# Mamo1031/Multimodal-MTRSSM

Hardware: AMD Instinct MI355X
Metric: seq-steps/s (BxT) MoPoE-MRSSM train step (higher is better)
Workload: dtype bf16x2-split, fp32 accumulate; 1 GPU; BASELINE configs[1]: MoPoE-MRSSM train step, B=64/GPU T=50 deter=200 stoch=30, vision 1x64x64 + audio 1x128x32 + action 4; global_batch=64, seq_len=50, parallelism=dp1, hidden=200, embed=256, categoricals_x_classes=6x5, residual_blocks=3, activation=ELU, optimizer=AdamW lr 1e-3 + clip 10 (fused HIP), params=4151600, streams=1, launch=eager (host enqueues every launch), backend=none, rccl_ranks=0, collective_ranks=0, noise=uniforms keyed by global batch row (parallel.GlobalRowNoise)

## Files before the change

include/mtrssm.h:

```cpp
#ifndef MTRSSM_H
#define MTRSSM_H

#include <stddef.h>
#include <stdint.h>

#ifdef __cplusplus
extern "C" {
#endif

#define MTRSSM_VERSION 100

#define MTRSSM_OK 0
#define MTRSSM_EINVAL (-1)
#define MTRSSM_ELAUNCH (-2)
#define MTRSSM_ELDS (-3)

#define MTRSSM_ACT_IDENTITY 0
#define MTRSSM_ACT_RELU 1
#define MTRSSM_ACT_ELU 2
#define MTRSSM_ACT_TANH 3

int mtrssm_version(void);
const char* mtrssm_last_error(void);
const char* mtrssm_last_kernel(void);
// ... 388 lines not shown
                                 int64_t workspace_a_bytes, const MtrssmConvGeom* gb, const float* ab, const float* srcb, float* dwpb,
                                 float* dbiasb, void* workspace_b, int64_t workspace_b_bytes, int32_t defer, void* stream);
int mtrssm_conv_weight_grad_src_bias(const MtrssmConvGeom* g, const float* a, const float* src, int32_t pre_act_a, float* dwp,
                                     float* dsrc_bias, void* workspace, int64_t workspace_bytes, int32_t defer, void* stream);
int64_t mtrssm_conv_weight_grad_workspace_bytes(const MtrssmConvGeom* g, int32_t pre_act_a);
int mtrssm_unpack_conv_grads(const int64_t* table, int32_t count, int32_t blocks_per_entry, void* stream);
int mtrssm_convt_quad_supported(const MtrssmConvGeom* g4);
int mtrssm_convt_quad(const MtrssmConvGeom* ga4, const float* srca, const uint16_t* const* wqa4, const float* biasa, const float* actgrada,
                      float* outa, const MtrssmConvGeom* gb4, const float* srcb, const uint16_t* const* wqb4, const float* biasb,
                      const float* actgradb, float* outb, void* stream);
int mtrssm_convt_k4s2_thin(int32_t N, int32_t C, int32_t Hs, int32_t Ws, int32_t Cout, const float* src, const float* w,
                           const float* bias, int32_t pre_act, int32_t act, float* out, void* stream);
int mtrssm_convt_k4s2_band_supported(int32_t N, int32_t C, int32_t Hs, int32_t Ws, int32_t Cout);
int mtrssm_convt_k4s2_band(int32_t N, int32_t C, int32_t Hs, int32_t Ws, int32_t Cout, const float* src, const float* w,
                           const float* bias, int32_t pre_act, int32_t act, float* out, void* stream);
int mtrssm_conv_tgather_thin(int32_t N, int32_t O, int32_t Hs, int32_t Ws, int32_t Cout, int32_t KH, int32_t KW, int32_t stride, int32_t pad,
                             int32_t Ho, int32_t Wo, const float* y, const float* w, const float* bias, int32_t pre_act, int32_t act,
                             const float* actgrad_in, const float* add_in, float* out, void* stream);
int mtrssm_channel_sum(const float* x, int32_t N, int32_t C, int32_t HW, float* out, void* stream);

int mtrssm_episode_gather(const float* store, const int64_t* idx, const float* noise, int64_t n_episodes, int64_t B, int64_t T,
                          int64_t Tfull, int64_t E, float std_, float* input, float* target, void* stream);
int mtrssm_episode_gather_window(const float* store, const int64_t* idx, const int32_t* start, const float* noise, int64_t n_episodes,
                                 int64_t B, int64_t T, int64_t Tfull, int64_t E, float std_, float* input, float* target, void* stream);
int mtrssm_episode_gather_ragged(const float* store, const int64_t* idx, const int32_t* start, const int32_t* lengths, const float* noise,
                                 int64_t n_episodes, int64_t B, int64_t T, int64_t Tfull, int64_t E, float std_, float* input, float* target,
                                 int32_t* valid_out, void* stream);
int mtrssm_episode_gather_seeded(const float* store, const int64_t* idx, const int32_t* start, const int32_t* lengths, int32_t* valid_out,
                                 uint32_t key0, uint32_t key1, uint32_t epoch, int64_t n_episodes, int64_t B, int64_t T, int64_t Tfull,
                                 int64_t E, float std_, float* input, float* target, void* stream);
// ... 184 lines not shown
```

multimodal_mtrssm_amd/_lib.py:

```python

from __future__ import annotations

import ctypes as C
import os
from pathlib import Path

import torch
from torch import Tensor

_HERE = Path(__file__).resolve().parent
LIB_PATH = _HERE / "libmtrssm_hip.so"

ACT_IDS = {"Identity": 0, "ReLU": 1, "ELU": 2, "Tanh": 3}

_f = C.c_float
_i = C.c_int32
_p = C.c_void_p


def _struct(name: str, fields: list[tuple[str, type]]) -> type:
    return type(name, (C.Structure,), {"_fields_": fields})


def _ptrs(*names: str) -> list[tuple[str, type]]:
# ... 44 lines not shown
    "sv_l1", "sv_h1", "sv_la", "sv_lv", "expert_logw", "modality"))
MmtrssmBwdWeights = _struct("MtrssmMmtrssmBwdWeights", _ptrs(
    "wxl_s_t", "wdl", "wxh_t", "wdh", "wl1", "wh1", "wlp2", "wa2", "wv2", "whp2", "whq2"))
MmtrssmBwdIO = _struct("MtrssmMmtrssmBwdIO", _ptrs(
    "deter_l0", "deter_h0", "deter_l", "deter_h", "prior_logits_l", "prior_logits_h", "post_logits_l", "post_logits_h",
    "sv_l1", "sv_h1", "sv_la", "sv_lv",
    "g_deter_l", "g_deter_h", "g_hidden_l", "g_hidden_h", "g_post_stoch_l", "g_post_stoch_h", "g_prior_stoch_l",
    "g_prior_stoch_h", "g_post_logits_l", "g_post_logits_h", "g_prior_logits_l", "g_prior_logits_h", "g_kl_l", "g_kl_h",
    "g_deter_l0", "g_deter_h0", "g_hidden_l0", "g_hidden_h0", "g_stoch_l0", "g_stoch_h0",
    "d_ul", "d_uh", "d_zl1", "d_zh1", "d_lpl", "d_la", "d_lv", "d_lph", "d_lqh", "expert_logw", "g_expert_logw", "modality"))

ConvGeom = _struct("MtrssmConvGeom", [(n, _i) for n in (
    "N", "C", "Hs", "Ws", "C2", "Cpad", "KH", "KW", "SS", "TS", "OFFY", "OFFX", "Hq", "Wq", "OS", "QY", "QX", "Ho", "Wo",
    "Cout", "CoutPad", "pre_act", "act", "mfma_split")])

Gemm = _struct("MtrssmGemm", _ptrs("A", "B", "C", "bias", "zgrad", "colsum") + [(n, _i) for n in (
    "M", "N", "R", "lda", "ldb", "ldc", "ldz", "a_rmajor", "b_rmajor", "act_a", "act_b", "act_out", "act_z", "accumulate", "split_r")]
    + [("tickets", _p), ("n_tickets", _i), ("mfma_split", _i)])

ElboSchedule = _struct("MtrssmElboSchedule", [(n, _f) for n in ("c0", "c1", "free0", "free1", "w_a", "w_v", "beta_start", "warmup")])

STATE_MAX = 6
StateTable = _struct("MtrssmStateTable", [
    ("count", _i), ("width", _i * STATE_MAX), ("src_stride", C.c_int64 * STATE_MAX), ("src", _p * STATE_MAX), ("alt", _p * STATE_MAX),
    ("dst", _p * STATE_MAX)])

PANEL_COLUMNS = {"prior": 0, "observation": 1, "posterior": 2, "error": 3}
PanelGeom = _struct("MtrssmPanelGeom", [(n, _i) for n in ("N", "T", "Ca", "Ha", "Wa", "Cv", "Hv", "Wv", "scale", "gap", "bar", "label", "frame0")]
                    + [("columns", _i * 4), ("n_columns", _i), ("blank_unseen", _i)])

SYMBOLS: dict[str, tuple[type | None, list[type]]] = {
# ... 39 lines not shown
    "mtrssm_residual_bwd1x1": (C.c_int, [C.POINTER(ConvGeom), _p, _p, _p, _p, _p, _p, _p, C.c_int64, _i, _p]),
    "mtrssm_conv_weight_grad_src_bias_supported": (C.c_int, [C.POINTER(ConvGeom), _i]),
    "mtrssm_conv_weight_grad_src_bias": (C.c_int, [C.POINTER(ConvGeom), _p, _p, _i, _p, _p, _p, C.c_int64, _i, _p]),
    "mtrssm_conv_weight_grad_reduce": (C.c_int, [_p]),
    "mtrssm_conv_weight_grad_workspace_bytes": (C.c_int64, [C.POINTER(ConvGeom), _i]),
    "mtrssm_residual_bwd1x1_pair_supported": (C.c_int, [C.POINTER(ConvGeom), C.POINTER(ConvGeom)]),
    "mtrssm_residual_bwd1x1_pair": (C.c_int, [C.POINTER(ConvGeom), _p, _p, _p, _p, _p, _p, _p, C.c_int64,
                                              C.POINTER(ConvGeom), _p, _p, _p, _p, _p, _p, _p, C.c_int64, _i, _p]),
    "mtrssm_conv_weight_grad_pair_supported": (C.c_int, [C.POINTER(ConvGeom), C.POINTER(ConvGeom)]),
    "mtrssm_conv_weight_grad_pair": (C.c_int, [C.POINTER(ConvGeom), _p, _p, _p, _p, _p, C.c_int64,
                                               C.POINTER(ConvGeom), _p, _p, _p, _p, _p, C.c_int64, _i, _p]),
    "mtrssm_channel_sum": (C.c_int, [_p, _i, _i, _i, _p, _p]),
    "mtrssm_convt_k4s2_thin": (C.c_int, [_i, _i, _i, _i, _i, _p, _p, _p, _i, _i, _p, _p]),
    "mtrssm_convt_k4s2_band_supported": (C.c_int, [_i, _i, _i, _i, _i]),
    "mtrssm_convt_k4s2_band": (C.c_int, [_i, _i, _i, _i, _i, _p, _p, _p, _i, _i, _p, _p]),
    "mtrssm_convt_quad_supported": (C.c_int, [C.POINTER(ConvGeom)]),
    "mtrssm_convt_quad": (C.c_int, [C.POINTER(ConvGeom), _p, C.POINTER(C.c_void_p), _p, _p, _p, C.POINTER(ConvGeom), _p, C.POINTER(C.c_void_p),
                                    _p, _p, _p, _p]),
    "mtrssm_conv_tgather_thin": (C.c_int, [_i] * 11 + [_p, _p, _p, _i, _i, _p, _p, _p, _p]),
    "mtrssm_episode_gather": (C.c_int, [_p, _p, _p, C.c_int64, C.c_int64, C.c_int64, C.c_int64, C.c_int64, _f, _p, _p, _p]),
    "mtrssm_episode_gather_window": (C.c_int, [_p, _p, _p, _p, C.c_int64, C.c_int64, C.c_int64, C.c_int64, C.c_int64, _f, _p, _p, _p]),
    "mtrssm_state_select": (C.c_int, [C.POINTER(StateTable), _p, C.c_int64, _p]),
    "mtrssm_state_save": (C.c_int, [C.POINTER(StateTable), C.c_int64, C.c_int64, _p]),
    "mtrssm_state_save_at": (C.c_int, [C.POINTER(StateTable), _p, C.c_int64, C.c_int64, _p]),
    "mtrssm_episode_gather_ragged": (C.c_int, [_p, _p, _p, _p, _p, C.c_int64, C.c_int64, C.c_int64, C.c_int64, C.c_int64, _f, _p, _p, _p, _p]),
    "mtrssm_episode_gather_seeded": (C.c_int, [_p, _p, _p, _p, _p, C.c_uint32, C.c_uint32, C.c_uint32, C.c_int64, C.c_int64, C.c_int64, C.c_int64,
                                               C.c_int64, _f, _p, _p, _p]),
    "mtrssm_step_mask_ragged": (C.c_int, [_p, _p, C.c_int64, C.c_int64, C.c_int64, _f, _f, C.c_int64, C.c_int64, _p, _p, _p, _p, _p, _p, _p, _p]),
    "mtrssm_step_mask_forecast": (C.c_int, [_p, _p, _p, C.c_int64, C.c_int64, C.c_int64, _f, _f, C.c_int64, C.c_int64, C.c_int64, C.c_int64, _p, _p, _p,
                                            _p, _p, _p, _p, _p, _p]),
# ... 174 lines not shown
```

multimodal_mtrssm_amd/cnn.py:

```python

from __future__ import annotations

from typing import Any

import torch
from torch import Tensor, nn

from multimodal_mtrssm_amd import _lib
from multimodal_mtrssm_amd.linear import SPLIT_MIN_FLOPS, linear, linear_group
from multimodal_mtrssm_amd.conv import (
    gemm_pieces,
    conv2d,
    conv2d_pair,
    conv_transpose2d,
    conv_transpose2d_pair,
    residual_block,
    residual_block_pair,
)


def _act(name: str) -> nn.Module:
    return getattr(nn, name)()


def _cfg(config: Any) -> dict[str, Any]:
    return dict(config) if isinstance(config, dict) else dict(vars(config))


def _conv(x: Tensor, m: nn.Conv2d, *, pre_act: bool, act: int, coords: Tensor | None = None) -> Tensor:
    return conv2d(x, m.weight, m.bias, stride=m.stride[0], padding=m.padding[0], pre_act=pre_act, act=act, coords=coords)
# ... 39 lines not shown


def _conv_pair(xa: Tensor, ma: nn.Conv2d, ca: Tensor | None, xb: Tensor, mb: nn.Conv2d, cb: Tensor | None, *, pre_act: bool,
               act_a: int, act_b: int) -> tuple[Tensor, Tensor]:
    if _same_layer(ma, mb) and act_a == act_b:
        return conv2d_pair((xa, ma.weight, ma.bias, ma.stride[0], ma.padding[0], pre_act, act_a, ca),
                           (xb, mb.weight, mb.bias, mb.stride[0], mb.padding[0], pre_act, act_b, cb))
    return _conv(xa, ma, pre_act=pre_act, act=act_a, coords=ca), _conv(xb, mb, pre_act=pre_act, act=act_b, coords=cb)


def encode_pair(enc_a: "Encoder", enc_b: "Encoder", xa: Tensor, xb: Tensor) -> tuple[Tensor, Tensor]:
    lead_a, lead_b = xa.shape[:-3], xb.shape[:-3]
    xa, ca = enc_a.prepare(xa)
    xb, cb = enc_b.prepare(xb)
    if len(enc_a.convs) == len(enc_b.convs) and (enc_a.res_in is None) == (enc_b.res_in is None):
        for i, (ma, mb) in enumerate(zip(enc_a.convs, enc_b.convs, strict=True)):
            xa, xb = _conv_pair(xa, ma, ca if i == 0 else None, xb, mb, cb if i == 0 else None, pre_act=i > 0, act_a=enc_a.act_id,
                                act_b=enc_b.act_id)
        if enc_a.res_in is not None:
            xa, xb = _conv_pair(xa, enc_a.res_in, None, xb, enc_b.res_in, None, pre_act=True, act_a=enc_a.act_id, act_b=enc_b.act_id)
    else:
        xa, xb = enc_a.stem_convs(xa, ca), enc_b.stem_convs(xb, cb)
    xa, xb = _res_pair(enc_a.res, enc_b.res, xa, xb)
    return enc_a.head(xa, lead_a), enc_b.head(xb, lead_b)


def decode_pair(dec_a: "Decoder", dec_b: "Decoder", fa: Tensor, fb: Tensor, *, raw: bool = False) -> tuple[Tensor, Tensor]:
    lead_a, lead_b = fa.shape[:-1], fb.shape[:-1]
    first_a = first_b = None
    if len(dec_a.linears) > 0 and len(dec_b.linears) > 0 and all(
            2.0 * f.numel() * d.linears[0].weight.shape[0] < SPLIT_MIN_FLOPS for f, d in ((fa, dec_a), (fb, dec_b))):
        first_a, first_b = linear_group([(f.reshape(-1, f.shape[-1]), d.linears[0].weight, d.linears[0].bias, 0)
                                         for f, d in ((fa, dec_a), (fb, dec_b))])
# ... 59 lines not shown

    def forward(self, x: Tensor) -> Tensor:
        lead = x.shape[:-3]
        x = self.stem(x)
        for blk in self.res:
            x = blk(x)
        return self.head(x, lead)

    def prepare(self, x: Tensor) -> tuple[Tensor, Tensor | None]:
        if len(self.linears) == 0:
            self.materialize(tuple(x.shape[-3:]))
            self.to(x.device)
        x = x.reshape(-1, *x.shape[-3:]).float()
        return x, (self._coord_channels(x) if self.coord_conv else None)

    def stem_convs(self, x: Tensor, coords: Tensor | None) -> Tensor:
        for i, conv in enumerate(self.convs):
            x = _conv(x, conv, pre_act=i > 0, act=self.act_id, coords=coords if i == 0 else None)
        if self.res_in is not None:
            x = _conv(x, self.res_in, pre_act=True, act=self.act_id)
        return x

    def stem(self, x: Tensor) -> Tensor:
        return self.stem_convs(*self.prepare(x))

    def head(self, x: Tensor, lead: torch.Size) -> Tensor:
        x = x.flatten(start_dim=1)
        for lin in self.linears:
            x = linear(x, lin.weight, lin.bias, pre_act=self.act_id, pieces=gemm_pieces())
        return self.out_act(x).reshape(*lead, -1)


class Decoder(nn.Module):
# ... 63 lines not shown
```

multimodal_mtrssm_amd/conv.py:

```python

from __future__ import annotations

import ctypes as C
import os
import weakref

import torch
from torch import Tensor

from multimodal_mtrssm_amd import _lib
from multimodal_mtrssm_amd.linear import grad_target, grad_target_owner


def _pad_to(n: int, m: int) -> int:
    return (n + m - 1) // m * m


def _pads(cout: int, cin: int) -> tuple[int, int]:
    return _pad_to(cout, 64 if cout > 32 else 32), _pad_to(cin, 16)


_PACK_BUFFERS: dict[tuple, tuple[Tensor, Tensor | None]] = {}

PAIR_LAUNCH = os.environ.get("MTRSSM_PAIR_LAUNCH", "1") != "0"
# ... 228 lines not shown
        fa, ba = _job_work(ja)
        fb, bb = _job_work(jb)
        _lib.check(_lib.TIMERS.call("mtrssm_conv_gather_gemm_pair", lib.mtrssm_conv_gather_gemm_pair, *_job_args(ja), *_job_args(jb),
                                    _lib.stream_ptr(ja[1].device), flops=fa + fb, nbytes=ba + bb), "mtrssm_conv_gather_gemm_pair")
    return ra, rb


def _conv_forward_gather(x: Tensor, coords: Tensor | None, w: Tensor, bias: Tensor | None, stride: int, pad: int,
                         pre_act: bool, act: int, actgrad_in: Tensor | None = None, add_in: Tensor | None = None) -> Tensor:
    n, c, hs, ws = x.shape
    o, i, kh, kw = w.shape
    c2 = 0 if coords is None else coords.shape[0]
    if i != c + c2:
        msg = f"weight expects {i} input channels, got {c}+{c2}"
        raise ValueError(msg)
    ho = (hs + 2 * pad - kh) // stride + 1
    wo = (ws + 2 * pad - kw) // stride + 1
    wpq = pack_weight(w)
    wp = wpq[0]
    out = torch.empty(n, o, ho, wo, device=x.device, dtype=torch.float32)
    geom = _geom(N=n, C=c, Hs=hs, Ws=ws, C2=c2, Cpad=wp.shape[2], KH=kh, KW=kw, SS=stride, TS=1, OFFY=-pad, OFFX=-pad,
                 Hq=ho, Wq=wo, OS=1, QY=0, QX=0, Ho=ho, Wo=wo, Cout=o, CoutPad=wp.shape[0], pre_act=int(pre_act), act=act)
    _gather_gemm(geom, x, coords, wpq, bias, actgrad_in, out, add_in)
    return out


def _conv_transposed_gather(y: Tensor, w: Tensor, bias: Tensor | None, stride: int, pad: int, out_hw: tuple[int, int],
                            pre_act: bool, act: int, actgrad_in: Tensor | None = None, add_in: Tensor | None = None) -> Tensor:
    n, o, hs, ws = y.shape
    o2, c, kh, kw = w.shape
    if o2 != o:
        msg = f"weight expects {o2} gathered channels, got {o}"
        raise ValueError(msg)
    ho, wo = out_hw
    out = torch.empty(n, c, ho, wo, device=y.device, dtype=torch.float32)
    if (stride == 2 and kh == 4 and kw == 4 and pad == 1 and c <= 2 and (ho, wo) == (2 * hs, 2 * ws) and actgrad_in is None
            and add_in is None and o * ((8 + 2) * (32 + 2) + 1) * 4 <= 64 * 1024):
        lib = _lib.load()
        wc = w.contiguous()
# ... 649 lines not shown
```

multimodal_mtrssm_amd/csrc/capi.hip:

```cpp
#include <stdarg.h>
#include <stdio.h>

#include "scan_common.h"

namespace mtrssm {

static thread_local char g_err[512] = "";
static thread_local const char* g_kernel = "";

void set_last_kernel(const char* name) { g_kernel = name; }

void set_error(const char* fmt, ...) {
  va_list ap;
  va_start(ap, fmt);
  vsnprintf(g_err, sizeof(g_err), fmt, ap);
  va_end(ap);
}

int mrssm_fwd_launch(const MtrssmMrssmDims*, const MtrssmMrssmFwdWeights*, const MtrssmMrssmFwdIO*, hipStream_t);
int mrssm_bwd_launch(const MtrssmMrssmDims*, const MtrssmMrssmBwdWeights*, const MtrssmMrssmBwdIO*, hipStream_t);
int mmtrssm_fwd_launch(const MtrssmMmtrssmDims*, const MtrssmMmtrssmFwdWeights*, const MtrssmMmtrssmFwdIO*, hipStream_t);
int mmtrssm_bwd_launch(const MtrssmMmtrssmDims*, const MtrssmMmtrssmBwdWeights*, const MtrssmMmtrssmBwdIO*, hipStream_t);
int conv_gather_gemm_launch(const MtrssmConvGeom*, const float*, const float*, const float*, const unsigned short*, const float*, const float*, const float*, float*, hipStream_t);
int episode_gather_launch(const float*, const int64_t*, const float*, int64_t, int64_t, int64_t, int64_t, int64_t, float, float*, float*, hipStream_t);
// ... 32 lines not shown
int conv_residual_bwd1x1_supported(const MtrssmConvGeom*);
int conv_residual_bwd1x1_launch(const MtrssmConvGeom*, const float*, const float*, const unsigned short*, float*, float*, float*, void*, size_t, int,
                                hipStream_t);
int conv_residual_bwd1x1_pair_supported(const MtrssmConvGeom*, const MtrssmConvGeom*);
int conv_residual_bwd1x1_pair_launch(const MtrssmConvGeom*, const float*, const float*, const unsigned short*, float*, float*, float*, void*, size_t,
                                     const MtrssmConvGeom*, const float*, const float*, const unsigned short*, float*, float*, float*, void*, size_t, int,
                                     hipStream_t);
int conv_weight_grad_pair_supported(const MtrssmConvGeom*, const MtrssmConvGeom*);
int conv_weight_grad_pair_launch(const MtrssmConvGeom*, const float*, const float*, float*, float*, void*, size_t, const MtrssmConvGeom*, const float*,
                                 const float*, float*, float*, void*, size_t, int, hipStream_t);
int conv_weight_grad_src_bias_supported(const MtrssmConvGeom*, int);
int conv_weight_grad_src_bias_launch(const MtrssmConvGeom*, const float*, const float*, int, float*, float*, void*, size_t, int, hipStream_t);
int channel_sum_launch(const float*, int, int, int, float*, hipStream_t);
int convt_k4s2_band_supported(int, int, int, int, int);
int convt_k4s2_band_launch(int, int, int, int, int, const float*, const float*, const float*, int, int, float*, hipStream_t);
int convt_k4s2_thin_launch(int, int, int, int, int, const float*, const float*, const float*, int, int, float*, hipStream_t);
int conv_convt_quad_supported(const MtrssmConvGeom*);
int conv_convt_quad_launch(const MtrssmConvGeom*, const float*, const unsigned short* const*, const float*, const float*, float*,
                           const MtrssmConvGeom*, const float*, const unsigned short* const*, const float*, const float*, float*, hipStream_t);
int conv_tgather_thin_launch(int, int, int, int, int, int, int, int, int, int, int, const float*, const float*, const float*, int, int, const float*,
                             const float*, float*, hipStream_t);
int categorical_sample_fwd_launch(const float*, const float*, int64_t, int, int, float*, float*, float*, hipStream_t);
int categorical_sample_bwd_launch(const float*, const float*, const float*, int64_t, int, int, float*, hipStream_t);
int elbo_combine_fwd_launch(const float*, const float*, const float*, const float*, int64_t, float, float, float*, float*, float*, float*, hipStream_t);
int elbo_combine_bwd_launch(const float*, const float*, const float*, const float*, int64_t, float, float, float*, float*, float*, float*, hipStream_t);
int nll_fwd_launch(const float*, const float*, int64_t, int64_t, int, float*, hipStream_t);
int nll_bwd_launch(const float*, const float*, const float*, int64_t, int64_t, int, float*, hipStream_t);
int nll_masked_fwd_launch(const float*, const float*, const float*, const float*, int64_t, int64_t, int, float*, hipStream_t);
int nll_masked_bwd_launch(const float*, const float*, const float*, const float*, const float*, int64_t, int64_t, int, float*, hipStream_t);
int ensemble_score_launch(const float*, const float*, const int32_t*, int64_t, int64_t, int64_t, int64_t, int, float*, float*, float*, float*, float*,
// ... 400 lines not shown
}
MTRSSM_API int mtrssm_conv_tgather_thin(int32_t N, int32_t O, int32_t Hs, int32_t Ws, int32_t Cout, int32_t KH, int32_t KW, int32_t stride,
                                        int32_t pad, int32_t Ho, int32_t Wo, const float* y, const float* w, const float* bias, int32_t pre_act,
                                        int32_t act, const float* actgrad_in, const float* add_in, float* out, void* stream) {
  return conv_tgather_thin_launch(N, O, Hs, Ws, Cout, KH, KW, stride, pad, Ho, Wo, y, w, bias, pre_act, act, actgrad_in, add_in, out,
                                  static_cast<hipStream_t>(stream));
}
MTRSSM_API int mtrssm_convt_quad_supported(const MtrssmConvGeom* g4) { return conv_convt_quad_supported(g4); }
MTRSSM_API int mtrssm_convt_quad(const MtrssmConvGeom* ga4, const float* srca, const uint16_t* const* wqa4, const float* biasa,
                                 const float* actgrada, float* outa, const MtrssmConvGeom* gb4, const float* srcb,
                                 const uint16_t* const* wqb4, const float* biasb, const float* actgradb, float* outb, void* stream) {
  return conv_convt_quad_launch(ga4, srca, reinterpret_cast<const unsigned short* const*>(wqa4), biasa, actgrada, outa, gb4, srcb,
                                reinterpret_cast<const unsigned short* const*>(wqb4), biasb, actgradb, outb,
                                static_cast<hipStream_t>(stream));
}
MTRSSM_API int mtrssm_convt_k4s2_band_supported(int32_t N, int32_t C, int32_t Hs, int32_t Ws, int32_t Cout) {
  return convt_k4s2_band_supported(N, C, Hs, Ws, Cout);
}
MTRSSM_API int mtrssm_convt_k4s2_band(int32_t N, int32_t C, int32_t Hs, int32_t Ws, int32_t Cout, const float* src, const float* w,
                                     const float* bias, int32_t pre_act, int32_t act, float* out, void* stream) {
  return convt_k4s2_band_launch(N, C, Hs, Ws, Cout, src, w, bias, pre_act, act, out, static_cast<hipStream_t>(stream));
}
MTRSSM_API int mtrssm_convt_k4s2_thin(int32_t N, int32_t C, int32_t Hs, int32_t Ws, int32_t Cout, const float* src, const float* w,
                                      const float* bias, int32_t pre_act, int32_t act, float* out, void* stream) {
  return convt_k4s2_thin_launch(N, C, Hs, Ws, Cout, src, w, bias, pre_act, act, out, static_cast<hipStream_t>(stream));
}

MTRSSM_API int mtrssm_ensemble_score(const float* pred, const float* target, const int32_t* valid, int64_t B, int64_t S, int64_t T, int64_t E,
                                     int32_t act, float* mean, float* ens, float* best, float* spread, float* se_samples, void* stream) {
  return ensemble_score_launch(pred, target, valid, B, S, T, E, act, mean, ens, best, spread, se_samples, static_cast<hipStream_t>(stream));
// ... 105 lines not shown
```

multimodal_mtrssm_amd/csrc/conv.hip:

```cpp
#include <map>
#include <mutex>
#include <unordered_map>
#include <utility>

#include "scan_common.h"

namespace mtrssm {

void set_error(const char* fmt, ...);
void set_last_kernel(const char* name);

using f32x16 = __attribute__((ext_vector_type(16))) float;

constexpr int kKC = 16;
constexpr int kTP = 128;
constexpr int kConvThreads = 256;

__device__ __forceinline__ float act_grad_from_in(float x, int act) {
  switch (act) {
    case MTRSSM_ACT_RELU: return x > 0.f ? 1.f : 0.f;
    case MTRSSM_ACT_ELU: return x > 0.f ? 1.f : expf(x);
    case MTRSSM_ACT_TANH: { const float t = tanhf(x); return 1.f - t * t; }
    default: return 1.f;
  }
// ... 546 lines not shown
            const size_t o = base + (size_t)co * plane_o;
            if (actgrad_in) v *= act_grad_from_in(actgrad_in[o], g.act);
            if (add_in) v += add_in[o];
            out[o] = v;
          }
        }
      }
    }
  }
}

}
#include "conv_split.h"
#include "conv_resident.h"
#include "conv_s2_band.h"
#include "conv_wgrad_resident.h"

namespace mtrssm {

static int launched(const char* who);
enum ReduceVariant { kRedRes64, kRedRes32, kRed1x1_64, kRed1x1_128, kRedThin, kRedThinT, kRedS2, kRedT4, kRedT4b, kRedS2c };
struct ReduceJob {
  const float4* part;
  float* dwp;
  float* dbias;
  int S, cpad, variant, gx, gy;
  __host__ int variant_gy() const { return gy; }
};
constexpr int kReduceBatchMax = 48;
struct ReduceBatch {
// ... 1844 lines not shown
  const int slots = 2 * cu_count();
  p.nx = N < slots ? N : slots;
  none.nx = 0;
  const size_t lds = (size_t)convt_band_lds_bytes(Hs, Ws);
  static bool attr_done_dev[64] = {};
  bool& attr_done = attr_done_dev[device_slot()];
  if (!attr_done) {
    (void)hipFuncSetAttribute(reinterpret_cast<const void*>(convt4s2_band_kernel), hipFuncAttributeMaxDynamicSharedMemorySize, 80 * 1024);
    attr_done = true;
  }
  set_last_kernel("mtrssm::convt4s2_band_kernel");
  hipLaunchKernelGGL(convt4s2_band_kernel, dim3((unsigned)p.nx), dim3(256), lds, stream, p, none);
  return launched("convt_k4s2_band");
}

int convt_k4s2_thin_launch(int N, int C, int Hs, int Ws, int Cout, const float* src, const float* w, const float* bias, int pre_act,
                           int act, float* out, hipStream_t stream) {
  if (N <= 0 || C <= 0 || Hs <= 0 || Ws <= 0 || Cout <= 0 || Cout > 2 || !src || !w || !out) {
    set_error("convt_k4s2_thin: bad argument (needs 1 <= Cout <= 2)");
    return MTRSSM_EINVAL;
  }
  if (act < MTRSSM_ACT_IDENTITY || act > MTRSSM_ACT_TANH) { set_error("convt_k4s2_thin: unknown activation id %d", act); return MTRSSM_EINVAL; }
  if ((uintptr_t)out & 7) { set_error("convt_k4s2_thin: out must be 8-byte aligned"); return MTRSSM_EINVAL; }
  const size_t lds = (size_t)C * kCtPS * sizeof(float);
  if (lds > 64 * 1024) { set_error("convt_k4s2_thin: %d input channels do not fit the LDS tile", C); return MTRSSM_ELDS; }
  const int tw = Ws <= 16 ? 16 : 32, th = kConvThreads / tw;
  const dim3 grid((Ws + tw - 1) / tw, (Hs + th - 1) / th, N);
#define MTRSSM_CT_LAUNCH(COT_, TW_)                                                                                  \
  { set_last_kernel("mtrssm::convt_k4s2_thin_kernel<" #COT_ ", " #TW_ ">"); hipLaunchKernelGGL((convt_k4s2_thin_kernel<COT_, TW_>), grid, dim3(kConvThreads), lds, stream, N, C, Hs, Ws, Cout, src, w, bias, pre_act, act, out); }
  if (Cout == 1) { if (tw == 16) MTRSSM_CT_LAUNCH(1, 16) else MTRSSM_CT_LAUNCH(1, 32) }
// ... 161 lines not shown
```

Baseline: 383,900 seq-steps/s.

## Fuse three-layer encoder conv stem into one persistent LDS-resident kernel

Adds a persistent kernel that runs the first three stride-2 3x3 convs of both encoders (vision and audio) in one launch. Each workgroup keeps one frame's intermediates in LDS and prefetches the next frame's input. The Python conv path then returns the outputs precomputed by this kernel. This removes separate launches and the global-memory round trips between stem layers, and it splits the CUs between the two modalities. The cost is a highly shape-specialised kernel (1+2 -> 8 -> 16 -> 32 channels, fixed plane sizes) and a global dict keyed by pointers that intercepts conv calls.

Result: faster. 388,900 seq-steps/s (median of 6 runs) (+1.3%).

```diff
diff --git a/include/mtrssm.h b/include/mtrssm.h
--- a/include/mtrssm.h
+++ b/include/mtrssm.h
@@ -426,6 +426,23 @@
 int mtrssm_convt_k4s2_band_supported(int32_t N, int32_t C, int32_t Hs, int32_t Ws, int32_t Cout);
 int mtrssm_convt_k4s2_band(int32_t N, int32_t C, int32_t Hs, int32_t Ws, int32_t Cout, const float* src, const float* w,
                            const float* bias, int32_t pre_act, int32_t act, float* out, void* stream);
+typedef struct MtrssmEncoderStem {
+  const float* src;
+  const float* coords;
+  const float* wp1;
+  const uint16_t* wq1;
+  const float* bias1;
+  const uint16_t* wq2;
+  const float* bias2;
+  const uint16_t* wq3;
+  const float* bias3;
+  float* y1;
+  float* y2;
+  float* y3;
+  int32_t N, C, C2, Hs, Ws, Cout1, Cout2, Cout3, act, mfma_split;
+} MtrssmEncoderStem;
+int mtrssm_encoder_stem_supported(const MtrssmEncoderStem* p);
+int mtrssm_encoder_stem_fwd(const MtrssmEncoderStem* a, const MtrssmEncoderStem* b, void* stream);
 int mtrssm_conv_tgather_thin(int32_t N, int32_t O, int32_t Hs, int32_t Ws, int32_t Cout, int32_t KH, int32_t KW, int32_t stride, int32_t pad,
                              int32_t Ho, int32_t Wo, const float* y, const float* w, const float* bias, int32_t pre_act, int32_t act,
                              const float* actgrad_in, const float* add_in, float* out, void* stream);
diff --git a/multimodal_mtrssm_amd/_lib.py b/multimodal_mtrssm_amd/_lib.py
--- a/multimodal_mtrssm_amd/_lib.py
+++ b/multimodal_mtrssm_amd/_lib.py
@@ -82,7 +82,11 @@
     "N", "C", "Hs", "Ws", "C2", "Cpad", "KH", "KW", "SS", "TS", "OFFY", "OFFX", "Hq", "Wq", "OS", "QY", "QX", "Ho", "Wo",
     "Cout", "CoutPad", "pre_act", "act", "mfma_split")])
 
-Gemm = _struct("MtrssmGemm", _ptrs("A", "B", "C", "bias", "zgrad", "colsum") + [(n, _i) for n in (
+EncoderStem = _struct("MtrssmEncoderStem", _ptrs(
+    "src", "coords", "wp1", "wq1", "bias1", "wq2", "bias2", "wq3", "bias3", "y1", "y2", "y3") + [(n, _i) for n in (
+    "N", "C", "C2", "Hs", "Ws", "Cout1", "Cout2", "Cout3", "act", "mfma_split")])
+
+Gemm = _struct("MtrssmGemm",_ptrs("A", "B", "C", "bias", "zgrad", "colsum") + [(n, _i) for n in (
     "M", "N", "R", "lda", "ldb", "ldc", "ldz", "a_rmajor", "b_rmajor", "act_a", "act_b", "act_out", "act_z", "accumulate", "split_r")]
     + [("tickets", _p), ("n_tickets", _i), ("mfma_split", _i)])
 
@@ -152,6 +156,8 @@
     "mtrssm_convt_k4s2_thin": (C.c_int, [_i, _i, _i, _i, _i, _p, _p, _p, _i, _i, _p, _p]),
     "mtrssm_convt_k4s2_band_supported": (C.c_int, [_i, _i, _i, _i, _i]),
     "mtrssm_convt_k4s2_band": (C.c_int, [_i, _i, _i, _i, _i, _p, _p, _p, _i, _i, _p, _p]),
+    "mtrssm_encoder_stem_supported": (C.c_int, [C.POINTER(EncoderStem)]),
+    "mtrssm_encoder_stem_fwd": (C.c_int, [C.POINTER(EncoderStem), C.POINTER(EncoderStem), _p]),
     "mtrssm_convt_quad_supported": (C.c_int, [C.POINTER(ConvGeom)]),
     "mtrssm_convt_quad": (C.c_int, [C.POINTER(ConvGeom), _p, C.POINTER(C.c_void_p), _p, _p, _p, C.POINTER(ConvGeom), _p, C.POINTER(C.c_void_p),
                                     _p, _p, _p, _p]),
diff --git a/multimodal_mtrssm_amd/cnn.py b/multimodal_mtrssm_amd/cnn.py
--- a/multimodal_mtrssm_amd/cnn.py
+++ b/multimodal_mtrssm_amd/cnn.py
@@ -14,6 +14,7 @@
     conv2d_pair,
     conv_transpose2d,
     conv_transpose2d_pair,
+    encoder_stem,
     residual_block,
     residual_block_pair,
 )
@@ -83,9 +84,10 @@
     xa, ca = enc_a.prepare(xa)
     xb, cb = enc_b.prepare(xb)
     if len(enc_a.convs) == len(enc_b.convs) and (enc_a.res_in is None) == (enc_b.res_in is None):
-        for i, (ma, mb) in enumerate(zip(enc_a.convs, enc_b.convs, strict=True)):
-            xa, xb = _conv_pair(xa, ma, ca if i == 0 else None, xb, mb, cb if i == 0 else None, pre_act=i > 0, act_a=enc_a.act_id,
-                                act_b=enc_b.act_id)
+        with encoder_stem([enc_a.stem_job(xa, ca), enc_b.stem_job(xb, cb)]):
+            for i, (ma, mb) in enumerate(zip(enc_a.convs, enc_b.convs, strict=True)):
+                xa, xb = _conv_pair(xa, ma, ca if i == 0 else None, xb, mb, cb if i == 0 else None, pre_act=i > 0, act_a=enc_a.act_id,
+                                    act_b=enc_b.act_id)
         if enc_a.res_in is not None:
             xa, xb = _conv_pair(xa, enc_a.res_in, None, xb, enc_b.res_in, None, pre_act=True, act_a=enc_a.act_id, act_b=enc_b.act_id)
     else:
@@ -175,9 +177,13 @@
         x = x.reshape(-1, *x.shape[-3:]).float()
         return x, (self._coord_channels(x) if self.coord_conv else None)
 
+    def stem_job(self, x: Tensor, coords: Tensor | None) -> tuple:
+        return x, coords, [(m.weight, m.bias, m.stride[0], m.padding[0]) for m in self.convs], self.act_id
+
     def stem_convs(self, x: Tensor, coords: Tensor | None) -> Tensor:
-        for i, conv in enumerate(self.convs):
-            x = _conv(x, conv, pre_act=i > 0, act=self.act_id, coords=coords if i == 0 else None)
+        with encoder_stem([self.stem_job(x, coords)]):
+            for i, conv in enumerate(self.convs):
+                x = _conv(x, conv, pre_act=i > 0, act=self.act_id, coords=coords if i == 0 else None)
         if self.res_in is not None:
             x = _conv(x, self.res_in, pre_act=True, act=self.act_id)
         return x
diff --git a/multimodal_mtrssm_amd/conv.py b/multimodal_mtrssm_amd/conv.py
--- a/multimodal_mtrssm_amd/conv.py
+++ b/multimodal_mtrssm_amd/conv.py
@@ -1,6 +1,7 @@
 
 from __future__ import annotations
 
+import contextlib
 import ctypes as C
 import os
 import weakref
@@ -266,6 +267,10 @@
     if i != c + c2:
         msg = f"weight expects {i} input channels, got {c}+{c2}"
         raise ValueError(msg)
+    if _STEM_FILLED is not None and actgrad_in is None and add_in is None:
+        out = _STEM_FILLED.pop((x.data_ptr(), w.data_ptr()), None)
+        if out is not None:
+            return out
     ho = (hs + 2 * pad - kh) // stride + 1
     wo = (ws + 2 * pad - kw) // stride + 1
     wpq = pack_weight(w)
@@ -275,6 +280,72 @@
                  Hq=ho, Wq=wo, OS=1, QY=0, QX=0, Ho=ho, Wo=wo, Cout=o, CoutPad=wp.shape[0], pre_act=int(pre_act), act=act)
     _gather_gemm(geom, x, coords, wpq, bias, actgrad_in, out, add_in)
     return out
+
+
+ENCODER_STEM = os.environ.get("MTRSSM_ENCODER_STEM", "1") != "0"
+_STEM_FILLED: dict[tuple[int, int], Tensor] | None = None
+
+
+def _stem_desc(x: Tensor, coords: Tensor | None, layers: list[tuple], act: int) -> C.Structure | None:
+    if not ENCODER_STEM or coords is None or len(layers) != 3 or x.dim() != 4 or x.dtype != torch.float32:
+        return None
+    if not (x.is_contiguous() and coords.is_contiguous() and coords.dim() == 3 and coords.shape[1:] == x.shape[2:]):
+        return None
+    if x.data_ptr() % 16 or coords.data_ptr() % 16 or coords.dtype != torch.float32:
+        return None
+    cin = x.shape[1] + coords.shape[0]
+    for w, b, stride, pad in layers:
+        if (tuple(w.shape[2:]) != (3, 3) or w.shape[1] != cin or stride != 2 or pad != 1 or not w.is_contiguous()
+                or (b is not None and not b.is_contiguous())):
+            return None
+        cin = w.shape[0]
+    p = _lib.EncoderStem()
+    p.N, p.C, p.Hs, p.Ws = (int(v) for v in x.shape)
+    p.C2 = int(coords.shape[0])
+    p.Cout1, p.Cout2, p.Cout3 = (int(w.shape[0]) for w, *_ in layers)
+    p.act, p.mfma_split = int(act), _MFMA_SPLIT
+    return p if _lib.load().mtrssm_encoder_stem_supported(C.byref(p)) else None
+
+
+def _stem_launch(jobs: list[tuple]) -> dict[tuple[int, int], Tensor]:
+    filled: dict[tuple[int, int], Tensor] = {}
+    flops = nbytes = 0.0
+    for k, (p, x, coords, layers) in enumerate(jobs):
+        n, _, h, w_ = x.shape
+        src, outs, packs = x, [], []
+        nbytes += 4.0 * x.numel()
+        for w, _b, _s, _p in layers:
+            packs.append(pack_weight(w, sub=100 + k))
+            h, w_ = h // 2, w_ // 2
+            out = torch.empty(n, w.shape[0], h, w_, device=x.device, dtype=torch.float32)
+            filled[(src.data_ptr(), w.data_ptr())] = out
+            flops += 2.0 * out.numel() * 9 * w.shape[1]
+            nbytes += 4.0 * out.numel()
+            outs.append(out)
+            src = out
+        p.src, p.coords = _lib.ptr(x), _lib.ptr(coords)
+        p.wp1, p.wq1, p.wq2, p.wq3 = _lib.ptr(packs[0][0]), _lib.raw_ptr(packs[0][1]), _lib.raw_ptr(packs[1][1]), _lib.raw_ptr(packs[2][1])
+        p.bias1, p.bias2, p.bias3 = (_lib.ptr(b) for _w, b, _s, _p in layers)
+        p.y1, p.y2, p.y3 = (_lib.ptr(o) for o in outs)
+    lib = _lib.load()
+    _lib.check(_lib.TIMERS.call("mtrssm_encoder_stem_fwd", lib.mtrssm_encoder_stem_fwd, C.byref(jobs[0][0]),
+                                C.byref(jobs[1][0]) if len(jobs) > 1 else None, _lib.stream_ptr(jobs[0][1].device), flops=flops,
+                                nbytes=nbytes), "mtrssm_encoder_stem_fwd")
+    return filled
+
+
+@contextlib.contextmanager
+def encoder_stem(jobs: list[tuple]):
+    global _STEM_FILLED
+    descs = [_stem_desc(x, coords, layers, act) if x.is_cuda else None for x, coords, layers, act in jobs]
+    if _STEM_FILLED is not None or not descs or len(descs) > 2 or any(d is None for d in descs):
+        yield False
+        return
+    _STEM_FILLED = _stem_launch([(d, x, coords, layers) for d, (x, coords, layers, _a) in zip(descs, jobs, strict=True)])
+    try:
+        yield True
+    finally:
+        _STEM_FILLED = None
 
 
 def _conv_transposed_gather(y: Tensor, w: Tensor, bias: Tensor | None, stride: int, pad: int, out_hw: tuple[int, int],
diff --git a/multimodal_mtrssm_amd/csrc/capi.hip b/multimodal_mtrssm_amd/csrc/capi.hip
--- a/multimodal_mtrssm_amd/csrc/capi.hip
+++ b/multimodal_mtrssm_amd/csrc/capi.hip
@@ -70,6 +70,8 @@
 int channel_sum_launch(const float*, int, int, int, float*, hipStream_t);
 int convt_k4s2_band_supported(int, int, int, int, int);
 int convt_k4s2_band_launch(int, int, int, int, int, const float*, const float*, const float*, int, int, float*, hipStream_t);
+int encoder_stem_supported(const MtrssmEncoderStem*);
+int encoder_stem_launch(const MtrssmEncoderStem*, const MtrssmEncoderStem*, hipStream_t);
 int convt_k4s2_thin_launch(int, int, int, int, int, const float*, const float*, const float*, int, int, float*, hipStream_t);
 int conv_convt_quad_supported(const MtrssmConvGeom*);
 int conv_convt_quad_launch(const MtrssmConvGeom*, const float*, const unsigned short* const*, const float*, const float*, float*,
@@ -500,6 +502,10 @@
                                 reinterpret_cast<const unsigned short* const*>(wqb4), biasb, actgradb, outb,
                                 static_cast<hipStream_t>(stream));
 }
+MTRSSM_API int mtrssm_encoder_stem_supported(const MtrssmEncoderStem* p) { return encoder_stem_supported(p); }
+MTRSSM_API int mtrssm_encoder_stem_fwd(const MtrssmEncoderStem* a, const MtrssmEncoderStem* b, void* stream) {
+  return encoder_stem_launch(a, b, static_cast<hipStream_t>(stream));
+}
 MTRSSM_API int mtrssm_convt_k4s2_band_supported(int32_t N, int32_t C, int32_t Hs, int32_t Ws, int32_t Cout) {
   return convt_k4s2_band_supported(N, C, Hs, Ws, Cout);
 }
diff --git a/multimodal_mtrssm_amd/csrc/conv.hip b/multimodal_mtrssm_amd/csrc/conv.hip
--- a/multimodal_mtrssm_amd/csrc/conv.hip
+++ b/multimodal_mtrssm_amd/csrc/conv.hip
@@ -584,6 +584,7 @@
 #include "conv_split.h"
 #include "conv_resident.h"
 #include "conv_s2_band.h"
+#include "conv_stem.h"
 #include "conv_wgrad_resident.h"
 
 namespace mtrssm {
@@ -2458,6 +2459,60 @@
   return launched("convt_k4s2_band");
 }
 
+int encoder_stem_supported(const MtrssmEncoderStem* p) {
+  return p && p->N > 0 && p->mfma_split == 2 && p->C == 1 && p->C2 == 2 && p->Cout1 == 8 && p->Cout2 == 16 && p->Cout3 == 32 &&
+                 ((p->Hs == 64 && p->Ws == 64) || (p->Hs == 128 && p->Ws == 32)) && p->act >= MTRSSM_ACT_IDENTITY && p->act < MTRSSM_ACT_TANH &&
+                 (long)p->N * 8 * 1024 < (1L << 31)
+             ? 1
+             : 0;
+}
+int encoder_stem_launch(const MtrssmEncoderStem* a, const MtrssmEncoderStem* b, hipStream_t stream) {
+  auto fill = [](const MtrssmEncoderStem* p, StemProblem& q) {
+    if (!encoder_stem_supported(p)) {
+      set_error("encoder_stem_fwd: needs bf16x2, channels 1 + 2 -> 8 -> 16 -> 32, 64 x 64 or 128 x 32 planes and a non-Tanh activation");
+      return MTRSSM_EINVAL;
+    }
+    if (!p->src || !p->coords || !p->wp1 || !p->wq1 || !p->wq2 || !p->wq3 || !p->y1 || !p->y2 || !p->y3) {
+      set_error("encoder_stem_fwd: null pointer");
+      return MTRSSM_EINVAL;
+    }
+    if (((uintptr_t)p->src | (uintptr_t)p->coords | (uintptr_t)p->wp1 | (uintptr_t)p->wq1 | (uintptr_t)p->wq2 | (uintptr_t)p->wq3 | (uintptr_t)p->y1 |
+         (uintptr_t)p->y2 | (uintptr_t)p->y3) & 15) {
+      set_error("encoder_stem_fwd: tensors must be 16-byte aligned");
+      return MTRSSM_EINVAL;
+    }
+    q.src = p->src; q.coords = p->coords; q.wp1 = p->wp1; q.wq1 = p->wq1; q.wq2 = p->wq2; q.wq3 = p->wq3;
+    q.b1 = p->bias1; q.b2 = p->bias2; q.b3 = p->bias3; q.y1 = p->y1; q.y2 = p->y2; q.y3 = p->y3;
+    q.N = p->N; q.Ws = p->Ws; q.act = p->act;
+    return MTRSSM_OK;
+  };
+  StemProblem qa{}, qb{};
+  if (int rc = fill(a, qa)) return rc;
+  if (b) {
+    if (int rc = fill(b, qb)) return rc;
+  }
+  const long ta = qa.N, tb = b ? qb.N : 0;
+  const int slots = cu_count();
+  if (tb == 0) {
+    qa.nx = (int)(ta < slots ? ta : slots);
+    qb.nx = 0;
+  } else {
+    long na = (slots * ta + (ta + tb) / 2) / (ta + tb);
+    na = na < 1 ? 1 : (na > slots - 1 ? slots - 1 : na);
+    qa.nx = (int)(na < ta ? na : ta);
+    qb.nx = (int)(slots - na < tb ? slots - na : tb);
+  }
+  static bool attr_done_dev[64] = {};
+  bool& attr_done = attr_done_dev[device_slot()];
+  if (!attr_done) {
+    (void)hipFuncSetAttribute(reinterpret_cast<const void*>(encoder_stem_kernel), hipFuncAttributeMaxDynamicSharedMemorySize, kStemLds);
+    attr_done = true;
+  }
+  set_last_kernel("mtrssm::encoder_stem_kernel");
+  hipLaunchKernelGGL(encoder_stem_kernel, dim3((unsigned)(qa.nx + qb.nx)), dim3(kStemThreads), (size_t)kStemLds, stream, qa, qb);
+  return launched("encoder_stem_fwd");
+}
+
 int convt_k4s2_thin_launch(int N, int C, int Hs, int Ws, int Cout, const float* src, const float* w, const float* bias, int pre_act,
                            int act, float* out, hipStream_t stream) {
   if (N <= 0 || C <= 0 || Hs <= 0 || Ws <= 0 || Cout <= 0 || Cout > 2 || !src || !w || !out) {
diff --git a/multimodal_mtrssm_amd/csrc/conv_stem.h b/multimodal_mtrssm_amd/csrc/conv_stem.h
--- /dev/null
+++ b/multimodal_mtrssm_amd/csrc/conv_stem.h
@@ -0,0 +1,275 @@
+#pragma once
+#include <type_traits>
+
+namespace mtrssm {
+
+struct StemProblem {
+  const float* src;
+  const float* coords;
+  const float* wp1;
+  const unsigned short* wq1;
+  const unsigned short* wq2;
+  const unsigned short* wq3;
+  const float* b1;
+  const float* b2;
+  const float* b3;
+  float* y1;
+  float* y2;
+  float* y3;
+  int N, Ws, act, nx;
+};
+
+constexpr int kStemThreads = 512;
+constexpr int kStemPlane = 4096;
+constexpr int kStemF = 65 * 32 * 16;
+constexpr int kStemY1 = 2 * 65 * 18 * 16;
+constexpr int kStemY2 = 4 * 298 * 16;
+constexpr int kStemImg = kStemF + kStemY1 + kStemY2;
+constexpr int kStemA3 = 2 * 10 * 64 * 16;
+constexpr int kStemLds = kStemImg + kStemA3;
+
+__global__ __launch_bounds__(kStemThreads, 1) void encoder_stem_kernel(const StemProblem pa, const StemProblem pb) {
+  const bool second = blockIdx.x >= (unsigned)pa.nx;
+#define MTRSSM_PICK(f) (second ? pb.f : pa.f)
+  const float* __restrict__ src = MTRSSM_PICK(src);
+  const float* __restrict__ coords = MTRSSM_PICK(coords);
+  const float* __restrict__ wp1 = MTRSSM_PICK(wp1);
+  const unsigned short* __restrict__ wq1 = MTRSSM_PICK(wq1);
+  const unsigned short* __restrict__ wq2 = MTRSSM_PICK(wq2);
+  const unsigned short* __restrict__ wq3 = MTRSSM_PICK(wq3);
+  const float* __restrict__ b1 = MTRSSM_PICK(b1);
+  const float* __restrict__ b2 = MTRSSM_PICK(b2);
+  const float* __restrict__ b3 = MTRSSM_PICK(b3);
+  float* __restrict__ y1 = MTRSSM_PICK(y1);
+  float* __restrict__ y2 = MTRSSM_PICK(y2);
+  float* __restrict__ y3 = MTRSSM_PICK(y3);
+  const int N = MTRSSM_PICK(N), Ws = MTRSSM_PICK(Ws), act = MTRSSM_PICK(act), nwg = MTRSSM_PICK(nx);
+#undef MTRSSM_PICK
+  const int wg = second ? (int)blockIdx.x - pa.nx : (int)blockIdx.x;
+  const int wsh = 31 - __builtin_clz(Ws);
+  const int Hs = kStemPlane >> wsh;
+  const int W1 = Ws >> 1, q1 = wsh - 1, H1 = Hs >> 1;
+  const int W2 = Ws >> 2, q2 = wsh - 2, H2 = Hs >> 2;
+  const int W3 = Ws >> 3, q3 = wsh - 3;
+  const int RP1 = (2 * W2 + 2) * 16, IMG1 = (H1 + 1) * RP1;
+  const int PW2 = W2 + 1, HALF2 = ((H2 + 1) * PW2 + 1) * 16, IMG2 = 2 * HALF2;
+  const int tid = threadIdx.x, lane = tid & 63, wave = tid >> 6;
+  const int l16 = lane & 15, g = lane >> 4, il = lane & 31, kl = lane >> 5;
+  if (wg >= N) return;
+  extern __shared__ __attribute__((aligned(16))) unsigned char stem_lds[];
+  unsigned char* const F = stem_lds;
+  unsigned char* const Y1 = stem_lds + kStemF;
+  unsigned char* const Y2 = stem_lds + kStemF + kStemY1;
+  unsigned char* const A3 = stem_lds + kStemImg;
+  using f32x4v = __attribute__((ext_vector_type(4))) float;
+  constexpr size_t PIECE = (size_t)32 * 9 * 16;
+
+  bf16x8 a1m, a1s;
+  {
+    const int ty = g < 3 ? g : 0;
+    u16x8 m = u16x8{0, 0, 0, 0, 0, 0, 0, 0}, s = m;
+#pragma unroll
+    for (int tx = 0; tx < 3; ++tx) {
+      const size_t o = ((size_t)l16 * 9 + ty * 3 + tx) * 16;
+      const unsigned short h0 = wq1[o], h1 = wq1[PIECE + o];
+      m[tx] = g < 3 ? h0 : (unsigned short)0;
+      m[4 + tx] = m[tx];
+      s[tx] = g < 3 ? h1 : (unsigned short)0;
+    }
+    a1m = __builtin_bit_cast(bf16x8, m);
+    a1s = __builtin_bit_cast(bf16x8, s);
+  }
+  bf16x8 a2[5][2];
+#pragma unroll
+  for (int kb = 0; kb < 5; ++kb) {
+    const int tap = 2 * kb + kl;
+#pragma unroll
+    for (int s = 0; s < 2; ++s) {
+      u32x4 v = u32x4{0u, 0u, 0u, 0u};
+      if (tap < 9) v = *reinterpret_cast<const u32x4*>(wq2 + s * PIECE + ((size_t)il * 9 + tap) * 16);
+      a2[kb][s] = __builtin_bit_cast(bf16x8, v);
+    }
+  }
+  const int u3 = wave & 3, ct = wave >> 2;
+  unsigned char* const a3 = A3 + ((size_t)ct * 10 * 64 + lane) * 16;
+  if (u3 == 0) {
+#pragma unroll
+    for (int ss = 0; ss < 5; ++ss) {
+      const int tap = 2 * ss + (g >> 1);
+#pragma unroll
+      for (int s = 0; s < 2; ++s) {
+        u32x4 v = u32x4{0u, 0u, 0u, 0u};
+        if (tap < 9) v = *reinterpret_cast<const u32x4*>(wq3 + s * PIECE + ((size_t)(16 * ct + l16) * 9 + tap) * 16 + 8 * (g & 1));
+        *reinterpret_cast<u32x4*>(a3 + (2 * ss + s) * 64 * 16) = v;
+      }
+    }
+  }
+  for (int o = tid * 16; o < kStemImg; o += kStemThreads * 16) *reinterpret_cast<u32x4*>(stem_lds + o) = u32x4{0u, 0u, 0u, 0u};
+
+  const int hi = g >> 1, gc = g & 1;
+  const int j0 = 128 * wave + l16, oy0 = j0 >> q1, ox0 = j0 & (W1 - 1);
+  auto doy = [&](int i) { return (16 * i) >> q1; };
+  auto dox = [&](int i) { return (16 * i) & (W1 - 1); };
+  const unsigned fa0 = (unsigned)(((2 * oy0 + (g < 3 ? g : 2)) * W1 + ox0) * 16);
+  auto fa = [&](int i) { return fa0 + (unsigned)((2 * doy(i) * W1 + dox(i)) * 16); };
+  const int ic0 = ox0 + 1;
+  const unsigned ya0 = (unsigned)((1 + oy0) * RP1 + ((ic0 & 1) ? W2 + 1 + (ic0 >> 1) : (ic0 >> 1)) * 16 + 8 * gc);
+  auto ya = [&](int i) { return ya0 + (unsigned)(doy(i) * RP1 + (dox(i) >> 1) * 16); };
+  f32x4v sv[8];
+#pragma unroll
+  for (int i = 0; i < 8; ++i) {
+    const int oy = oy0 + doy(i), ox = ox0 + dox(i);
+#pragma unroll
+    for (int r = 0; r < 4; ++r) sv[i][r] = b1 ? b1[(4 * g + r) & 7] : 0.f;
+#pragma unroll 1
+    for (int t = 0; t < 9; ++t) {
+      const int sy = 2 * oy - 1 + t / 3, sx = 2 * ox - 1 + t % 3;
+      const bool in = sy >= 0 && sy < Hs && sx >= 0 && sx < Ws;
+      const int so = in ? sy * Ws + sx : 0;
+      const float c0 = in ? coords[so] : 0.f, c1 = in ? coords[kStemPlane + so] : 0.f;
+#pragma unroll
+      for (int r = 0; r < 4; ++r) {
+        const float* w = wp1 + ((size_t)((4 * g + r) & 7) * 9 + t) * 16;
+        sv[i][r] = fmaf(w[2], c1, fmaf(w[1], c0, sv[i][r]));
+      }
+    }
+  }
+  unsigned ba2[5];
+  const int j2 = 32 * wave + il, oy2 = j2 >> q2, ox2 = j2 & (W2 - 1);
+#pragma unroll
+  for (int kb = 0; kb < 5; ++kb) {
+    const int tap = 2 * kb + kl < 9 ? 2 * kb + kl : 8, ty = tap / 3, tx = tap - 3 * ty;
+    const int slot = (tx & 1) ? W2 + 1 + ox2 : ox2 + (tx >> 1);
+    ba2[kb] = (unsigned)((2 * oy2 + ty) * RP1 + slot * 16);
+  }
+  const unsigned yb = (unsigned)(((oy2 + 1) * PW2 + ox2 + 1) * 16 + 8 * kl);
+  float bv2[8];
+#pragma unroll
+  for (int r = 0; r < 8; ++r) bv2[r] = b2 ? b2[4 * kl + (r & 3) + 8 * (r >> 2)] : 0.f;
+  const int j3 = 16 * u3 + l16, oy3 = j3 >> q3, ox3 = j3 & (W3 - 1);
+  unsigned ba3[5];
+#pragma unroll
+  for (int ss = 0; ss < 5; ++ss) {
+    const int tap = 2 * ss + (g >> 1) < 9 ? 2 * ss + (g >> 1) : 8, ty = tap / 3, tx = tap - 3 * ty;
+    ba3[ss] = (unsigned)((g & 1) * HALF2 + ((2 * oy3 + ty) * PW2 + 2 * ox3 + tx) * 16);
+  }
+  f32x4v bv3;
+#pragma unroll
+  for (int r = 0; r < 4; ++r) bv3[r] = b3 ? b3[16 * ct + 4 * g + r] : 0.f;
+
+  band_f4 pv[2];
+  auto request = [&](int n) {
+    const float* f = src + (size_t)n * kStemPlane;
+#pragma unroll
+    for (int k = 0; k < 2; ++k) pv[k] = *reinterpret_cast<const band_f4*>(f + (tid + kStemThreads * k) * 4);
+  };
+  auto stage = [&]() {
+#pragma unroll
+    for (int k = 0; k < 2; ++k) {
+      const int p = (tid + kStemThreads * k) * 4, r = p >> wsh, x = p & (Ws - 1);
+      const band_f4 v = pv[k];
+      float left = __shfl_up(v[3], 1);
+      if (x == 0) left = 0.f;
+      unsigned short hl[2], h[4][2];
+      split_bf16<2>(left, hl);
+#pragma unroll
+      for (int e = 0; e < 4; ++e) split_bf16<2>(v[e], h[e]);
+      const u16x8 qa = u16x8{hl[0], h[0][0], h[1][0], 0, hl[1], h[0][1], h[1][1], 0};
+      const u16x8 qb = u16x8{h[1][0], h[2][0], h[3][0], 0, h[1][1], h[2][1], h[3][1], 0};
+      unsigned char* d = F + ((r + 1) * W1 + (x >> 1)) * 16;
+      *reinterpret_cast<u16x8*>(d) = qa;
+      *reinterpret_cast<u16x8*>(d + 16) = qb;
+    }
+  };
+
+  auto frame = [&](int n, auto mode_tag) {
+    constexpr int MODE = decltype(mode_tag)::value;
+    auto activate = [&](float v) { return MODE == 1 ? elu_fast(v) : act_fwd(v, act); };
+    {
+      f32x4v acc[8];
+#pragma unroll
+      for (int hh = 0; hh < 2; ++hh) {
+        bf16x8 b[4];
+#pragma unroll
+        for (int i = 0; i < 4; ++i) b[i] = *reinterpret_cast<const bf16x8*>(F + fa(4 * hh + i));
+#pragma unroll
+        for (int i = 0; i < 4; ++i) acc[4 * hh + i] = __builtin_amdgcn_mfma_f32_16x16x32_bf16(a1s, b[i], sv[4 * hh + i], 0, 0, 0);
+#pragma unroll
+        for (int i = 0; i < 4; ++i) acc[4 * hh + i] = __builtin_amdgcn_mfma_f32_16x16x32_bf16(a1m, b[i], acc[4 * hh + i], 0, 0, 0);
+      }
+      float* o = y1 + (size_t)n * (8 * 1024) + (size_t)(4 * gc) * 1024 + j0 + 64 * hi;
+#pragma unroll
+      for (int i = 0; i < 4; ++i) {
+        unsigned short h[4][2];
+#pragma unroll
+        for (int r = 0; r < 4; ++r) {
+          const float up = __shfl(acc[i + 4][r], lane & 31);
+          const float v = hi ? up : acc[i][r];
+          o[r * 1024 + 16 * i] = v;
+          split_bf16<2>(activate(v), h[r]);
+        }
+        unsigned char* d = Y1 + (hi ? ya(i + 4) : ya(i));
+        *reinterpret_cast<uint2*>(d) = make_uint2((unsigned)h[0][0] | ((unsigned)h[1][0] << 16), (unsigned)h[2][0] | ((unsigned)h[3][0] << 16));
+        *reinterpret_cast<uint2*>(d + IMG1) = make_uint2((unsigned)h[0][1] | ((unsigned)h[1][1] << 16), (unsigned)h[2][1] | ((unsigned)h[3][1] << 16));
+      }
+    }
+    lds_barrier();
+    {
+      f32x16 acc;
+#pragma unroll
+      for (int r = 0; r < 16; ++r) acc[r] = r < 8 ? bv2[r] : 0.f;
+#pragma unroll
+      for (int kb = 0; kb < 5; ++kb) {
+        const bf16x8 b0 = *reinterpret_cast<const bf16x8*>(Y1 + ba2[kb]);
+        const bf16x8 b1q = *reinterpret_cast<const bf16x8*>(Y1 + ba2[kb] + IMG1);
+        acc = __builtin_amdgcn_mfma_f32_32x32x16_bf16(a2[kb][0], b1q, acc, 0, 0, 0);
+        acc = __builtin_amdgcn_mfma_f32_32x32x16_bf16(a2[kb][1], b0, acc, 0, 0, 0);
+        acc = __builtin_amdgcn_mfma_f32_32x32x16_bf16(a2[kb][0], b0, acc, 0, 0, 0);
+      }
+      float* o = y2 + (size_t)n * (16 * 256) + (size_t)(4 * kl) * 256 + j2;
+#pragma unroll
+      for (int hf = 0; hf < 2; ++hf) {
+        unsigned short h[4][2];
+#pragma unroll
+        for (int r = 0; r < 4; ++r) {
+          o[(8 * hf + r) * 256] = acc[4 * hf + r];
+          split_bf16<2>(activate(acc[4 * hf + r]), h[r]);
+        }
+        unsigned char* d = Y2 + hf * HALF2 + yb;
+        *reinterpret_cast<uint2*>(d) = make_uint2((unsigned)h[0][0] | ((unsigned)h[1][0] << 16), (unsigned)h[2][0] | ((unsigned)h[3][0] << 16));
+        *reinterpret_cast<uint2*>(d + IMG2) = make_uint2((unsigned)h[0][1] | ((unsigned)h[1][1] << 16), (unsigned)h[2][1] | ((unsigned)h[3][1] << 16));
+      }
+    }
+    lds_barrier();
+    {
+      f32x4v acc = bv3;
+#pragma unroll
+      for (int ss = 0; ss < 5; ++ss) {
+        const bf16x8 b0 = *reinterpret_cast<const bf16x8*>(Y2 + ba3[ss]);
+        const bf16x8 b1q = *reinterpret_cast<const bf16x8*>(Y2 + ba3[ss] + IMG2);
+        const bf16x8 w0 = *reinterpret_cast<const bf16x8*>(a3 + (2 * ss) * 64 * 16);
+        const bf16x8 w1 = *reinterpret_cast<const bf16x8*>(a3 + (2 * ss + 1) * 64 * 16);
+        acc = __builtin_amdgcn_mfma_f32_16x16x32_bf16(w0, b1q, acc, 0, 0, 0);
+        acc = __builtin_amdgcn_mfma_f32_16x16x32_bf16(w1, b0, acc, 0, 0, 0);
+        acc = __builtin_amdgcn_mfma_f32_16x16x32_bf16(w0, b0, acc, 0, 0, 0);
+      }
+      float* o = y3 + (size_t)n * (32 * 64) + (size_t)(16 * ct + 4 * g) * 64 + j3;
+#pragma unroll
+      for (int r = 0; r < 4; ++r) o[r * 64] = acc[r];
+    }
+  };
+
+  const int last = wg + ((N - 1 - wg) / nwg) * nwg;
+  request(wg);
+  __syncthreads();
+  for (int n = wg; n < N; n += nwg) {
+    stage();
+    const int nx = n + nwg;
+    request(nx < last ? nx : last);
+    lds_barrier();
+    if (act == MTRSSM_ACT_ELU) frame(n, std::integral_constant<int, 1>{});
+    else frame(n, std::integral_constant<int, 2>{});
+  }
+}
+
+}
```
